# HakimNessah/th_rl

Hardware: AMD Instinct MI355X
Metric: env-steps/sec, 2-agent PD x 1M parallel games (higher is better)
Workload: dtype f32

## Files before the change

th_rl_amd/csrc/thrl_wave_kernel.h:

```cpp
#pragma once
#include <type_traits>
#include "thrl_kernels.h"
#include "thrl_wave_lut.h"

#ifndef THRL_ABLATE
#define THRL_ABLATE 0
#endif

namespace thrl {

constexpr int kAblate = THRL_ABLATE;

typedef unsigned int v2u __attribute__((ext_vector_type(2)));

__device__ __forceinline__ v2u pack_halves(unsigned a, unsigned b) {
    return __builtin_amdgcn_permlane32_swap(a, b, false, false);
}

__device__ __forceinline__ unsigned lds_addr(const void* p) {
    return (unsigned)(uintptr_t)(__attribute__((address_space(3))) const void*)p;
}
template <typename QT>
__device__ __forceinline__ QT lds_load(unsigned addr) {
    typedef __attribute__((address_space(3))) QT lds_t;
    return *(const lds_t*)(uintptr_t)addr;
}
template <typename QT>
__device__ __forceinline__ void lds_store(unsigned addr, QT v) {
    typedef __attribute__((address_space(3))) QT lds_t;
    *(lds_t*)(uintptr_t)addr = v;
}

__device__ __forceinline__ unsigned bperm(unsigned byte_sel, unsigned v) {
    return (unsigned)__builtin_amdgcn_ds_bpermute((int)byte_sel, (int)v);
}

template <int CTRL>
__device__ __forceinline__ double dpp_mov64(double v) {
    const int lo = __double2loint(v), hi = __double2hiint(v);
    return __hiloint2double(__builtin_amdgcn_update_dpp(hi, hi, CTRL, 0xF, 0xF, false),
                            __builtin_amdgcn_update_dpp(lo, lo, CTRL, 0xF, 0xF, false));
}
template <int CTRL>
__device__ __forceinline__ uint32_t dpp_mov32(uint32_t v) {
    return (uint32_t)__builtin_amdgcn_update_dpp((int)v, (int)v, CTRL, 0xF, 0xF, false);
}

__device__ __forceinline__ float group8_allmax(float v) {
    asm("s_nop 1\n\t"
        "v_max_f32_dpp %0, %0, %0 quad_perm:[1,0,3,2] row_mask:0xf bank_mask:0xf\n\t"
        "s_nop 1\n\t"
        "v_max_f32_dpp %0, %0, %0 quad_perm:[2,3,0,1] row_mask:0xf bank_mask:0xf\n\t"
        "s_nop 1\n\t"
        "v_max_f32_dpp %0, %0, %0 row_half_mirror row_mask:0xf bank_mask:0xf"
        : "+v"(v));
    return v;
}
__device__ __forceinline__ double group8_allmax(double v) {
    v = fmax(v, dpp_mov64<0xB1>(v));
    v = fmax(v, dpp_mov64<0x4E>(v));
    v = fmax(v, dpp_mov64<0x141>(v));
    return v;
}
__device__ __forceinline__ void store_where(unsigned long long mask, unsigned addr, float v) {
    unsigned long long save;
    asm volatile("s_mov_b64 %0, exec\n\ts_mov_b64 exec, %1\n\tds_write_b32 %2, %3\n\ts_mov_b64 exec, %0"
                 : "=&s"(save) : "s"(mask), "v"(addr), "v"(v) : "memory");
}
__device__ __forceinline__ void store_where(unsigned long long mask, unsigned addr, double v) {
    unsigned long long save;
    asm volatile("s_mov_b64 %0, exec\n\ts_mov_b64 exec, %1\n\tds_write_b64 %2, %3\n\ts_mov_b64 exec, %0"
                 : "=&s"(save) : "s"(mask), "v"(addr), "v"(v) : "memory");
}
__device__ __forceinline__ float dpp_ror8(float v) { return __builtin_bit_cast(float, dpp_mov32<0x128>(__builtin_bit_cast(uint32_t, v))); }
__device__ __forceinline__ double dpp_ror8(double v) { return dpp_mov64<0x128>(v); }
__device__ __forceinline__ float max_of(float a, float b) { return fmaxf(a, b); }
__device__ __forceinline__ double max_of(double a, double b);
__device__ __forceinline__ float half32_allmax(float v) {
    v = group8_allmax(v);
    v = fmaxf(v, __builtin_bit_cast(float, dpp_mov32<0x140>(__builtin_bit_cast(uint32_t, v))));
    unsigned a = __builtin_bit_cast(unsigned, v), b = a;
    asm("" : "+v"(b));
    const v2u r = __builtin_amdgcn_permlane16_swap(a, b, false, false);
    const unsigned rx = r.x, ry = r.y;
    return fmaxf(__builtin_bit_cast(float, rx), __builtin_bit_cast(float, ry));
}
__device__ __forceinline__ double half32_allmax(double v) {
    v = group8_allmax(v);
    v = fmax(v, dpp_mov64<0x140>(v));
    unsigned lo = (unsigned)__double2loint(v), hi = (unsigned)__double2hiint(v);
    unsigned lo2 = lo, hi2 = hi;
    asm("" : "+v"(lo2), "+v"(hi2));
    const v2u rl = __builtin_amdgcn_permlane16_swap(lo, lo2, false, false);
    const v2u rh = __builtin_amdgcn_permlane16_swap(hi, hi2, false, false);
    const unsigned rlx = rl.x, rly = rl.y, rhx = rh.x, rhy = rh.y;
    return fmax(__hiloint2double((int)rhx, (int)rlx), __hiloint2double((int)rhy, (int)rly));
}
__device__ __forceinline__ double max_of(double a, double b) { return fmax(a, b); }

__device__ __forceinline__ double wave_sum4(double q0, double q1, double q2, double q3, int lane) {
    const bool odd = lane & 1;
    const double k0 = odd ? q1 : q0, k1 = odd ? q3 : q2;
    const double s0 = odd ? q0 : q1, s1 = odd ? q2 : q3;
    const double a0 = k0 + dpp_mov64<0xB1>(s0);
    const double a1 = k1 + dpp_mov64<0xB1>(s1);
    const bool b1 = lane & 2;
    const double kk = b1 ? a1 : a0, ss = b1 ? a0 : a1;
    double v = kk + dpp_mov64<0x4E>(ss);
    v = v + dpp_mov64<0x124>(v);
    v = v + dpp_mov64<0x128>(v);
    {
        unsigned lo = (unsigned)__double2loint(v), hi = (unsigned)__double2hiint(v);
        unsigned lo2 = lo, hi2 = hi;
        asm("" : "+v"(lo2), "+v"(hi2));
        const v2u rl = __builtin_amdgcn_permlane16_swap(lo, lo2, false, false);
        const v2u rh = __builtin_amdgcn_permlane16_swap(hi, hi2, false, false);
        const unsigned rlx = rl.x, rly = rl.y, rhx = rh.x, rhy = rh.y;
        v = __hiloint2double((int)rhx, (int)rlx) + __hiloint2double((int)rhy, (int)rly);
    }
    {
        unsigned lo = (unsigned)__double2loint(v), hi = (unsigned)__double2hiint(v);
        unsigned lo2 = lo, hi2 = hi;
        asm("" : "+v"(lo2), "+v"(hi2));
        const v2u rl = __builtin_amdgcn_permlane32_swap(lo, lo2, false, false);
        const v2u rh = __builtin_amdgcn_permlane32_swap(hi, hi2, false, false);
        const unsigned rlx = rl.x, rly = rl.y, rhx = rh.x, rhy = rh.y;
        v = __hiloint2double((int)rhx, (int)rlx) + __hiloint2double((int)rhy, (int)rly);
    }
    return v;
}

template <int CTRL>
__device__ __forceinline__ uint32_t dpp_src(uint32_t v) {
    return (uint32_t)__builtin_amdgcn_update_dpp(0, (int)v, CTRL, 0xF, 0xF, true);
}

__device__ __forceinline__ float max3_f32(float a, float b, float c) {
    float r;
    asm("v_max3_f32 %0, %1, %2, %3" : "=v"(r) : "v"(a), "v"(b), "v"(c));
    return r;
}
__device__ __forceinline__ uint32_t argmax21_first(unsigned row) {
    float g[7];
#pragma unroll
    for (int k = 0; k < 7; k++)
        g[k] = max3_f32(lds_load<float>(row + 12u * k), lds_load<float>(row + 12u * k + 4u), lds_load<float>(row + 12u * k + 8u));
    const float m = max3_f32(max3_f32(g[0], g[1], g[2]), max3_f32(g[3], g[4], g[5]), g[6]);
    uint32_t c3 = 18u;
#pragma unroll
    for (int k = 5; k >= 0; k--) c3 = (g[k] == m) ? (uint32_t)(3 * k) : c3;
    const unsigned ad = row + 4u * c3;
    const float va = lds_load<float>(ad), vb = lds_load<float>(ad + 4u);
    uint32_t pos = (vb == m) ? 1u : 2u;
    pos = (va == m) ? 0u : pos;
    const float v0 = lds_load<float>(row);
    return (v0 != v0) ? 0u : c3 + pos;
}

__device__ __forceinline__ uint32_t readlane_u(uint32_t v, int lane) {
    return (uint32_t)__builtin_amdgcn_readlane((int)v, lane);
}

__device__ __forceinline__ uint32_t writelane_u(uint32_t old, uint32_t val, int lane) {
    asm("s_mov_b32 m0, %2\n\ts_nop 0\n\tv_writelane_b32 %0, %1, m0" : "+v"(old) : "s"(val), "s"(lane));
    return old;
}

__device__ __forceinline__ uint32_t halves_sum(uint32_t x) {
    uint32_t y;
    asm("v_add_u32_sdwa %0, %1, %1 dst_sel:DWORD dst_unused:UNUSED_PAD src0_sel:WORD_0 src1_sel:WORD_1" : "=v"(y) : "v"(x));
    return y;
}

template <int T0>
__device__ __forceinline__ void chain_group(uint32_t& sq, int& s, uint32_t n0, uint32_t n1, uint32_t n2, uint32_t n3) {
    int s1, s2, s3, s4, pk;
    asm volatile(
        "s_nop 3\n\t"
        "v_readlane_b32 %1, %7, %6\n\t"
        "s_pack_ll_b32_b16 %5, %6, %1\n\t"
        "v_writelane_b32 %0, %5, %11\n\t"
        "s_nop 1\n\t"
        "v_readlane_b32 %2, %8, %1\n\t"
        "s_nop 3\n\t"
        "v_readlane_b32 %3, %9, %2\n\t"
        "s_pack_ll_b32_b16 %5, %2, %3\n\t"
        "v_writelane_b32 %0, %5, %12\n\t"
        "s_nop 1\n\t"
        "v_readlane_b32 %4, %10, %3"
        : "+v"(sq), "=&s"(s1), "=&s"(s2), "=&s"(s3), "=&s"(s4), "=&s"(pk)
        : "s"(s), "v"(n0), "v"(n1), "v"(n2), "v"(n3), "n"(T0), "n"(T0 + 2)
        : "scc");
    s = s4;
}

template <int T0>
__device__ __forceinline__ void chain_group_greedy(uint32_t& sq, int& s, uint32_t g1, uint32_t g2, uint32_t g3, uint32_t g4) {
    int s1, s2, s3, s4, pk;
    asm volatile(
        "s_nop 3\n\t"
        "v_readlane_b32 %1, %7, %6\n\t"
        "v_readlane_b32 %2, %8, %6\n\t"
        "v_readlane_b32 %3, %9, %6\n\t"
        "v_readlane_b32 %4, %10, %6\n\t"
        "s_pack_ll_b32_b16 %5, %6, %1\n\t"
        "v_writelane_b32 %0, %5, %11\n\t"
        "s_pack_ll_b32_b16 %5, %2, %3\n\t"
        "v_writelane_b32 %0, %5, %12"
        : "+v"(sq), "=&s"(s1), "=&s"(s2), "=&s"(s3), "=&s"(s4), "=&s"(pk)
        : "s"(s), "v"(g1), "v"(g2), "v"(g3), "v"(g4), "n"(T0), "n"(T0 + 2)
        : "scc");
    s = s4;
}

template <bool ON> struct GreedyTables {
    __device__ __forceinline__ void build(unsigned) {}
    template <int T0> __device__ __forceinline__ void chain(uint32_t&, int&) const {}
};
template <> struct GreedyTables<true> {
    uint32_t g1, g2, g3, g4;
    __device__ __forceinline__ void build(unsigned lut_addr) {
        g1 = (uint32_t)lds_load<unsigned short>(lut_addr);
        g2 = bperm((g1 & 63u) << 2, g1);
        g3 = bperm((g2 & 63u) << 2, g1);
        g4 = bperm((g2 & 63u) << 2, g2);
    }
    template <int T0> __device__ __forceinline__ void chain(uint32_t& sq, int& s) const { chain_group_greedy<T0>(sq, s, g1, g2, g3, g4); }
};

template <int NRSEG>
__device__ __forceinline__ uint32_t read_row(const uint32_t (&r)[NRSEG], int s) {
    uint32_t v = readlane_u(r[0], s & 63);
    if (NRSEG > 1) {
        const uint32_t h = readlane_u(r[NRSEG - 1], s & 63);
        if (s >= 64) v = h;
    }
    return v;
}
template <int NRSEG>
__device__ __forceinline__ uint32_t gather_row(const uint32_t (&r)[NRSEG], uint32_t row) {
    uint32_t v = bperm((row & 63u) << 2, r[0]);
    if (NRSEG > 1) {
        const uint32_t h = bperm((row & 63u) << 2, r[NRSEG - 1]);
        if (row >= 64u) v = h;
    }
    return v;
}

template <typename QT> struct BlockOps;
template <> struct BlockOps<float> {
    unsigned c1;
    __device__ __forceinline__ void permute(unsigned sel) { c1 = bperm(sel, c1); }
    __device__ __forceinline__ void keep() const { asm volatile("" :: "v"(c1)); }
    __device__ __forceinline__ float value(float nm, float alpha_gamma, float, float) const {
        return __fmaf_rn(alpha_gamma, nm, __builtin_bit_cast(float, c1));
    }
};
template <> struct BlockOps<double> {
    unsigned r_lo, r_hi, t4_lo, t4_hi;
    __device__ __forceinline__ void keep() const { asm volatile("" :: "v"(r_lo), "v"(r_hi), "v"(t4_lo), "v"(t4_hi)); }
    __device__ __forceinline__ void permute(unsigned sel) {
        r_lo = bperm(sel, r_lo); r_hi = bperm(sel, r_hi); t4_lo = bperm(sel, t4_lo); t4_hi = bperm(sel, t4_hi);
    }
    __device__ __forceinline__ double value(double nm, double, double alpha, double gamma) const {
        const double re = __hiloint2double((int)r_hi, (int)r_lo), t4 = __hiloint2double((int)t4_hi, (int)t4_lo);
        const double t2 = __dadd_rn(re, __dmul_rn(gamma, nm));
        return __dadd_rn(t4, __dmul_rn(alpha, t2));
    }
};
template <typename QT> struct Snapshot;
template <> struct Snapshot<float> {
    v2u t4;
    __device__ __forceinline__ void set(float oma0, float ov0, float oma1, float ov1) {
        t4 = pack_halves(__builtin_bit_cast(unsigned, __fmul_rn(oma0, ov0)), __builtin_bit_cast(unsigned, __fmul_rn(oma1, ov1)));
    }
};
template <> struct Snapshot<double> {
    v2u lo, hi;
    __device__ __forceinline__ void set(double oma0, double ov0, double oma1, double ov1) {
        const double x0 = __dmul_rn(oma0, ov0), x1 = __dmul_rn(oma1, ov1);
        lo = pack_halves((unsigned)__double2loint(x0), (unsigned)__double2loint(x1));
        hi = pack_halves((unsigned)__double2hiint(x0), (unsigned)__double2hiint(x1));
    }
};
__device__ __forceinline__ BlockOps<float> make_ops(const Snapshot<float>& s, int k, double r0d, double r1d, float alpha_h) {
    const v2u req = pack_halves(__builtin_bit_cast(unsigned, (float)r0d), __builtin_bit_cast(unsigned, (float)r1d));
    BlockOps<float> o;
    o.c1 = __builtin_bit_cast(unsigned, __fmaf_rn(alpha_h, __builtin_bit_cast(float, k ? req.y : req.x),
                                                  __builtin_bit_cast(float, k ? s.t4.y : s.t4.x)));
    return o;
}
__device__ __forceinline__ BlockOps<double> make_ops(const Snapshot<double>& s, int k, double r0d, double r1d, double) {
    const v2u rl = pack_halves((unsigned)__double2loint(r0d), (unsigned)__double2loint(r1d));
    const v2u rh = pack_halves((unsigned)__double2hiint(r0d), (unsigned)__double2hiint(r1d));
    BlockOps<double> o;
    o.r_lo = k ? rl.y : rl.x; o.r_hi = k ? rh.y : rh.x;
    o.t4_lo = k ? s.lo.y : s.lo.x; o.t4_hi = k ? s.hi.y : s.hi.x;
    return o;
}
template <typename QT> struct HP;
template <> struct HP<float> {
    static __device__ __forceinline__ float gamma(const AgentParams& p) { return p.gamma_f; }
    static __device__ __forceinline__ float alpha(const AgentParams& p) { return p.alpha_f; }
    static __device__ __forceinline__ float one_minus_alpha(const AgentParams& p) { return p.one_minus_alpha_f; }
    static __device__ __forceinline__ float from_double(double x) { return (float)x; }
    static __device__ __forceinline__ float product(float a, float g) { return __fmul_rn(a, g); }
};
template <> struct HP<double> {
    static __device__ __forceinline__ double gamma(const AgentParams& p) { return p.gamma; }
    static __device__ __forceinline__ double alpha(const AgentParams& p) { return p.alpha; }
    static __device__ __forceinline__ double one_minus_alpha(const AgentParams& p) { return p.one_minus_alpha; }
    static __device__ __forceinline__ double from_double(double x) { return x; }
    static __device__ __forceinline__ double product(double, double) { return 0.0; }
};

template <typename QT, int RDN, bool FIXED_POINTS, bool PER2>
__device__ __forceinline__ void replay_group(int gi, uint32_t P, int lane_base, int nsub, const BlockOps<QT>& ops, unsigned wo,
                                             unsigned rd_base, unsigned row_shift, unsigned my_step,
                                             unsigned row_bytes, QT alpha_gamma, QT alpha, QT gamma, bool upper_half,
                                             int block_step0, int replay_from) {
    const int first = replay_from - (block_step0 + gi * 4);
    if (first >= 4) return;
    const uint32_t sP = readlane_u(P, lane_base + gi * 4);
    const int nv = min(4, nsub - gi * 4);
    unsigned ad0;
    asm("v_mad_u32_u24 %0, %1, %2, %3" : "=v"(ad0) : "v"((sP >> row_shift) & 0x7Fu), "s"(row_bytes), "v"(rd_base));
    unsigned ad[RDN];
#pragma unroll
    for (int i = 0; i < RDN; i++) ad[i] = ad0 + (unsigned)(i * sizeof(QT));
    if (FIXED_POINTS && PER2 && (sP >> 31) && nv == 4 && first <= 0 && !(kAblate & 256) && (sP & 0x7Fu) != ((sP >> 7) & 0x7Fu)) {
        const unsigned ca0 = readlane_u(wo, gi), ca1 = readlane_u(wo, 32 + gi);
        const unsigned cb0 = readlane_u(wo, 8 + gi), cb1 = readlane_u(wo, 40 + gi);
        const bool odd = (my_step & 1u) != 0u;
// ... 261 lines not shown
        if (SWEEP && a.sw_gamma) gamma_h = HP<QT>::from_double(a.sw_gamma[(size_t)half * a.G + g]);
        if (SWEEP && a.sw_alpha) {
            alpha_h = HP<QT>::from_double(a.sw_alpha[(size_t)half * a.G + g]);
            oma0 = HP<QT>::from_double(__dsub_rn(1.0, a.sw_alpha[g]));
            oma1 = HP<QT>::from_double(__dsub_rn(1.0, a.sw_alpha[(size_t)a.G + g]));
        }
        double epsg0 = 0.0, epsg1 = 0.0;
        const bool sw_eps_on = SWEEP && a.sw_eps != nullptr;
        if (sw_eps_on) { epsg0 = a.sw_eps[g]; epsg1 = a.sw_eps[(size_t)a.G + g]; }
        const QT ag_h = HP<QT>::product(alpha_h, gamma_h);
        const double eend0 = (SWEEP && a.sw_eps_end) ? a.sw_eps_end[g] : p0.eps_end;
        const double eend1 = (SWEEP && a.sw_eps_end) ? a.sw_eps_end[(size_t)a.G + g] : p1.eps_end;
        const double estep0 = (SWEEP && a.sw_eps_step) ? a.sw_eps_step[g] : p0.eps_step;
        const double estep1 = (SWEEP && a.sw_eps_step) ? a.sw_eps_step[(size_t)a.G + g] : p1.eps_step;
        const double noise_prob_g = (SWEEP && a.sw_noise_prob) ? a.sw_noise_prob[g] : a.env.noise_prob;

        {
            const QT* s0 = q0 + lo * A;
            const QT* s1 = q1 + lo * A;
            const int n = W * A;
            for (int k0 = 0; k0 < n; k0 += 512) {
                QT v0[8], v1[8];
#pragma unroll
                for (int j = 0; j < 8; j++) {
                    const int k = min(k0 + j * 64 + lane, n - 1);
                    v0[j] = s0[k]; v1[j] = s1[k];
                }
#pragma unroll
                for (int j = 0; j < 8; j++) {
                    const int k = k0 + j * 64 + lane;
                    if (k < n) { tab0[k] = v0[j]; tab1[k] = v1[j]; }
                }
            }
        }
        int sp = __builtin_amdgcn_readfirstlane(encode32(price0, p0));
        int st = __builtin_amdgcn_readfirstlane(encode64(price0, p0));
        sp = min(max(sp, 0), a.rows - 1);
        st = min(max(st, 0), a.rows - 1);
        int spill0 = -1, spill1 = -1, sp_l, st_l;
        if (sp >= lo && sp < lo + W) sp_l = sp - lo; else { spill0 = sp; sp_l = W; }
        if (st == sp) st_l = sp_l;
        else if (st >= lo && st < lo + W) st_l = st - lo;
        else { spill1 = st; st_l = W + 1; }

        {
            if (spill0 >= 0 && lane < A) {
                tab0[W * A + lane] = q0[spill0 * A + lane];
                tab1[W * A + lane] = q1[spill0 * A + lane];
            }
            if (spill1 >= 0 && lane < A) {
                tab0[(W + 1) * A + lane] = q0[spill1 * A + lane];
                tab1[(W + 1) * A + lane] = q1[spill1 * A + lane];
            }
        }
        __builtin_amdgcn_wave_barrier();

        int s = sp_l | (st_l << 8);
        double last_price = price0;
        for (int e = 0; e < a.n_episodes; e += epk) {
            const uint32_t eg = (uint32_t)(a.first_episode + (uint64_t)e);

            uint32_t AM[NRSEG], R[NRSEG];
            uint32_t G0q = 0u, G1q = 0u;
#pragma unroll
            for (int k = 0; k < NRSEG; k++) {
                const int row = min(lane + 64 * k, W + 1);
                const QT* r0 = tab0 + row * A;
                const QT* r1 = tab1 + row * A;
                QT b0 = r0[0], b1 = r1[0];
                uint32_t i0 = 0, i1 = 0;
                if (kAblate & 16) {
                } else if (kArgmax21 && A == 21) {
                    i0 = argmax21_first(tab0_off + (unsigned)row * 84u);
                    i1 = argmax21_first(tab1_off + (unsigned)row * 84u);
                } else if (A == 21) {
#pragma unroll
                    for (int j = 1; j < 21; j++) {
                        const QT v0 = r0[j], v1 = r1[j];
                        if (v0 > b0) { b0 = v0; i0 = j; }
                        if (v1 > b1) { b1 = v1; i1 = j; }
                    }
                } else {
#pragma unroll 4
                    for (int j = 1; j < A; j++) {
                        const QT v0 = r0[j], v1 = r1[j];
                        if (v0 > b0) { b0 = v0; i0 = j; }
                        if (v1 > b1) { b1 = v1; i1 = j; }
                    }
                }
                if (kAblate & 16) { i0 = (uint32_t)(lane * 5) % (uint32_t)A; i1 = (uint32_t)(lane * 3) % (uint32_t)A; }
                AM[k] = i0 | (i1 << 8);
                R[k] = (i0 * (uint32_t)A * 2u) | (i1 << 17);
                if constexpr (AFFINE) {
                    G0q = i0 * ((uint32_t)a.aff_m0 * 0x01010101u);
                    G1q = i1 * ((uint32_t)a.aff_m1 * 0x01010101u);
                }
            }
            GreedyTables<GREEDY && NRSEG == 1> gt;
            gt.build(halves_sum(R[0]) + lut_ns_lds);

            uint32_t seq[NSEG], rwv[NSEG];
            unsigned explored_segs = 0u;
            double nav[NSEG];
#pragma unroll
            for (int seg = 0; seg < NSEG; seg++) {
                int n = min(64, T - seg * 64);
                asm volatile("" : "+s"(n));
                uint32_t rw;
                nav[seg] = 0.0;
                const int tcl = min(seg * 64 + lane, T - 1);
                const int ep = epk == 1 ? 0 : tcl / Tenv;
                const uint32_t st_in_ep = (uint32_t)(tcl - ep * Tenv);
                double eps0, eps1;
                if (sw_eps_on) { eps0 = epsg0; eps1 = epsg1; }
                else if (epk == 1) { eps0 = a.eps[e][0]; eps1 = a.eps[e][1]; }
                else { eps0 = a.eps[e + ep][0]; eps1 = a.eps[e + ep][1]; }
                if (a.inj_u) {
                    const int tt = tcl;
                    const size_t k = (((size_t)e * Tenv + tt) * 2) * (size_t)a.G + (size_t)g;
                    const uint32_t ex0 = a.inj_u[k] < eps0 ? 1u : 0u;
                    const uint32_t ex1 = a.inj_u[k + a.G] < eps1 ? 2u : 0u;
                    const uint32_t c0 = min((uint32_t)(uint8_t)a.inj_choice[k], (uint32_t)(A - 1));
                    const uint32_t c1 = min((uint32_t)(uint8_t)a.inj_choice[k + a.G], (uint32_t)(A - 1));
                    rw = ex0 | ex1 | (c0 << 8) | (c1 << 16);
                } else if (kAblate & 8) {
                    const uint32_t h = (uint32_t)(lane * 2654435761u) ^ eg;
                    rw = (h & 3u) | (((h >> 4) % (uint32_t)A) << 8) | (((h >> 12) % (uint32_t)A) << 16);
                } else {
                    uint32_t seed_lo = (uint32_t)a.seed, seed_hi = (uint32_t)(a.seed >> 32);
                    asm volatile("" : "+s"(seed_lo), "+s"(seed_hi));
                    const uint64_t seed_here = ((uint64_t)seed_hi << 32) | seed_lo;
                    const u32x4 x = draw(seed_here, gid, eg + (uint32_t)ep, st_in_ep, 0u);
                    const uint32_t ex0 = u01_32(x.x) < eps0 ? 1u : 0u;
                    const uint32_t ex1 = u01_32(x.z) < eps1 ? 2u : 0u;
                    rw = ex0 | ex1 | (__umulhi(x.y, (uint32_t)A) << 8) | (__umulhi(x.w, (uint32_t)A) << 16);
                }
                if (NOISE) {
                    double nu, na;
                    if (a.inj_u) {
                        const size_t k = ((size_t)e * Tenv + tcl) * (size_t)a.G + (size_t)g;
                        nu = a.inj_noise_u[k]; na = a.inj_noise_a[k];
                    } else {
                        const u32x4 xn = draw(a.seed, gid, eg + (uint32_t)ep, st_in_ep, kStreamNoise);
                        nu = u01_32(xn.x);
                        na = __dadd_rn(a.env.noise_lo, __dmul_rn(__dsub_rn(a.env.a, a.env.noise_lo), u01_32(xn.y)));
                    }
                    if (nu < noise_prob_g) rw |= 4u;
                    nav[seg] = na;
                }
                rwv[seg] = rw;
                if constexpr (AFFINE) {
                    seq[seg] = play_affine(seg, n, lane, rw, G0q, G1q, mk_addr, a.aff_c, a.aff_m0, a.aff_m1, s);
                } else {
                const uint32_t Mv = ((rw & 1u) ? 0u : 0xFFFFu) | ((rw & 2u) ? 0u : 0xFFFF0000u);
                const uint32_t Kv = lut_ns_lds + 2u * (((rw & 1u) ? ((rw >> 8) & 0xFFu) * (uint32_t)A : 0u) +
                                                      ((rw & 2u) ? ((rw >> 16) & 0xFFu) : 0u));
                const unsigned long long noisy_steps = NOISE ? __ballot((rw & 4u) != 0u) : 0ull;
                unsigned long long busy_groups = 0ull;
                if (GREEDY && __ballot((rw & 3u) != 0u && seg * 64 + lane < T) != 0ull) explored_segs |= 1u << seg;
                if (GREEDY && NRSEG == 1) {
                    busy_groups = __ballot((rw & (NOISE ? 7u : 3u)) != 0u || seg * 64 + lane >= T);
                    busy_groups |= busy_groups >> 1;
                    busy_groups |= busy_groups >> 2;
                }
                constexpr bool greedy_copy = GREEDY && NRSEG == 1 && !(kAblate & 6);
                auto build = [&](int t, uint32_t (&out)[NRSEG], bool may_be_noisy) {
                    const int tl = t;
                    if (NOISE && may_be_noisy) {
                        if ((noisy_steps >> tl) & 1ull) {
                            const uint32_t w = readlane_u(rw, tl);
                            const double na = __hiloint2double(__builtin_amdgcn_readlane(__double2hiint(nav[seg]), tl),
                                                               __builtin_amdgcn_readlane(__double2loint(nav[seg]), tl));
                            const uint32_t c0 = (w >> 8) & 0xFFu, c1 = (w >> 16) & 0xFFu;
#pragma unroll
                            for (int k = 0; k < NRSEG; k++) {
                                const uint32_t a0r = (w & 1u) ? c0 : (AM[k] & 0xFFu), a1r = (w & 2u) ? c1 : (AM[k] >> 8);
                                const double Q = __dadd_rn(lut_aq[a0r], lut_aq[A + a1r]);
                                double pr = __dsub_rn(na, __dmul_rn(a.env.b, Q));
                                if (!(pr > 0.0)) pr = 0.0;
                                const int r32 = min(max(encode32_fast(pr, p0) - lo, 0), W - 1);
                                const int r64 = min(max(encode64_fast(pr, p0) - lo, 0), W - 1);
                                out[k] = (uint32_t)(r32 | (r64 << 8));
                            }
                            return;
                        }
                    }
                    if (kAblate & 4) {
#pragma unroll
                        for (int k = 0; k < NRSEG; k++) out[k] = (R[k] >> 17) + (uint32_t)(t & 3);
                        return;
                    }
                    const uint32_t sM = readlane_u(Mv, tl), sK = readlane_u(Kv, tl);
#pragma unroll
                    for (int k = 0; k < NRSEG; k++) out[k] = lds_load<unsigned short>(halves_sum(R[k] & sM) + sK);
                };
                uint32_t sq = 0, sq_tail = 0;
                auto chain4 = [&](auto t0c, const int n, const uint32_t (&tab)[4][NRSEG], const bool all_greedy = false) {
                    constexpr int t0 = decltype(t0c)::value;
                    if (kAblate & 2) {
                        asm volatile("" :: "v"(tab[0][0]), "v"(tab[1][0]), "v"(tab[2][0]), "v"(tab[3][0]));
                        sq_tail = (uint32_t)min(lane, W - 1) * 0x101u;
                        return;
                    }
                    if (NRSEG == 1 && t0 + 4 <= n) {
                        s = __builtin_amdgcn_readfirstlane(s);
                        if (GREEDY && all_greedy) gt.template chain<t0>(sq, s);
                        else chain_group<t0>(sq, s, tab[0][0], tab[1][0], tab[2][0], tab[3][0]);
                        return;
                    }
                    s = __builtin_amdgcn_readfirstlane(s);
#pragma unroll
                    for (int j = 0; j < 4; j++) {
                        if (t0 + j < n) {
                            sq_tail = writelane_u(sq_tail, (uint32_t)s, t0 + j);
                            s = (int)read_row<NRSEG>(tab[j], s & 0xFF);
                        }
                    }
                };
                uint32_t ta[4][NRSEG], tb[4][NRSEG];
                v2u mkr[4] = {v2u{0u, 0u}, v2u{0u, 0u}, v2u{0u, 0u}, v2u{0u, 0u}};
                if (kLdsMK) {
                    if (lane < 32) lds_store<v2u>(mk_addr + 8u * (unsigned)lane, v2u{Mv, Kv});
                    __builtin_amdgcn_wave_barrier();
#pragma unroll
                    for (int j = 0; j < 4; j++) mkr[j] = lds_load<v2u>(mk_addr + 8u * (unsigned)j);
                }
                auto build4 = [&](int t0, uint32_t (&tab)[4][NRSEG]) {
                    if (kLdsMK) {
                        unsigned ad[4];
#pragma unroll
                        for (int j = 0; j < 4; j++) ad[j] = halves_sum(R[0] & mkr[j].x) + mkr[j].y;
#pragma unroll
                        for (int j = 0; j < 4; j++) tab[j][0] = lds_load<unsigned short>(ad[j]);
                        if (t0 == 28) {
                            if (lane >= 32) lds_store<v2u>(mk_addr + 8u * (unsigned)(lane - 32), v2u{Mv, Kv});
                            __builtin_amdgcn_wave_barrier();
                        }
#pragma unroll
                        for (int j = 0; j < 4; j++) mkr[j] = lds_load<v2u>(mk_addr + 8u * (unsigned)(min(t0 + 4 + j, 63) & 31));
                        return;
                    }
                    if (NOISE && ((noisy_steps >> t0) & 0xFull)) {
#pragma unroll
                        for (int j = 0; j < 4; j++) build(t0 + j, tab[j], true);
                    } else {
#pragma unroll
                        for (int j = 0; j < 4; j++) build(t0 + j, tab[j], false);
                    }
                };
#define THRL_PLAY2(G, N_)                                                                    \
                if ((G) * 4 < (N_)) {                                                        \
                    if ((G) * 4 + 4 < (N_)) build4((G) * 4 + 4, tb);                         \
                    chain4(std::integral_constant<int, (G) * 4>(), (N_), ta);                \
                    if ((G) * 4 + 4 < (N_)) {                                                \
                        if ((G) * 4 + 8 < (N_)) build4((G) * 4 + 8, ta);                     \
                        chain4(std::integral_constant<int, (G) * 4 + 4>(), (N_), tb);        \
                    }                                                                        \
                }
#define THRL_PLAY16(N_)                                                                      \
                THRL_PLAY2(0, N_) THRL_PLAY2(2, N_) THRL_PLAY2(4, N_) THRL_PLAY2(6, N_)      \
                THRL_PLAY2(8, N_) THRL_PLAY2(10, N_) THRL_PLAY2(12, N_) THRL_PLAY2(14, N_)
#define THRL_PLAY2G(G, N_)                                                                   \
                if ((G) * 4 + 8 <= (N_) && g0 &&                                             \
                    !(busy_groups & (((G) * 4 + 8 < 64 ? 0x110ull : 0x10ull) << ((G) * 4)))) {   \
                     \
                    chain4(std::integral_constant<int, (G) * 4>(), (N_), ta, true);          \
                    chain4(std::integral_constant<int, (G) * 4 + 4>(), (N_), tb, true);      \
                } else if ((G) * 4 < (N_)) {                                                 \
                    const bool g1 = !((busy_groups >> ((G) * 4 + 4)) & 1ull);                \
                    if ((G) * 4 + 4 < (N_) && !g1) build4((G) * 4 + 4, tb);                  \
                    chain4(std::integral_constant<int, (G) * 4>(), (N_), ta, g0);            \
                    if ((G) * 4 + 4 < (N_)) {                                                \
                        g0 = (G) * 4 + 8 < 64 && !((busy_groups >> (((G) * 4 + 8) & 63)) & 1ull);   \
                        if ((G) * 4 + 8 < (N_) && !g0) build4((G) * 4 + 8, ta);              \
                        chain4(std::integral_constant<int, (G) * 4 + 4>(), (N_), tb, g1);    \
                    }                                                                        \
                }
#define THRL_PLAY16G(N_)                                                                         \
                THRL_PLAY2G(0, N_) THRL_PLAY2G(2, N_) THRL_PLAY2G(4, N_) THRL_PLAY2G(6, N_)      \
                THRL_PLAY2G(8, N_) THRL_PLAY2G(10, N_) THRL_PLAY2G(12, N_) THRL_PLAY2G(14, N_)
                if (greedy_copy) {
                    bool g0 = !(busy_groups & 1ull);
                    if (!g0) build4(0, ta);
                    if (n == 64) { THRL_PLAY16G(64) } else if (n == 36) { THRL_PLAY16G(36) } else { THRL_PLAY16G(n) }
                } else {
                    build4(0, ta);
                    if (n == 64) { THRL_PLAY16(64) } else if (n == 36) { THRL_PLAY16(36) } else { THRL_PLAY16(n) }
                }
#undef THRL_PLAY16G
#undef THRL_PLAY2G
#undef THRL_PLAY16
#undef THRL_PLAY2
                {
                    const int packed_end = (NRSEG == 1 && !(kAblate & 2)) ? (n & ~3) : 0;
                    const uint32_t prev = dpp_mov32<0x111>(sq);
                    const uint32_t un = (lane & 1) ? (prev >> 16) : (sq & 0xFFFFu);
                    seq[seg] = lane < packed_end ? un : sq_tail;
                }
                }
            }
            const int s_end = s;

            uint32_t act[NSEG];
            Snapshot<QT> snap[NSEG];
#pragma unroll
            for (int seg = 0; seg < NSEG; seg++) {
                const int tt = seg * 64 + lane;
                const bool valid = tt < T;
                const uint32_t my_s = seq[seg] & 0xFFu;
                const uint32_t my_train = (seq[seg] >> 8) & 0xFFu;
                const uint32_t rw = rwv[seg];
                const uint32_t gam = gather_row<NRSEG>(AM, my_s);
                uint32_t a0 = (rw & 1u) ? ((rw >> 8) & 0xFFu) : (gam & 0xFFu);
                uint32_t a1 = (rw & 2u) ? ((rw >> 16) & 0xFFu) : (gam >> 8);
                uint32_t nxt = (uint32_t)__shfl_down((int)seq[seg], 1, 64);
                if (seg + 1 < NSEG) { if (lane == 63) nxt = readlane_u(seq[seg + 1 < NSEG ? seg + 1 : seg], 0); }
                const uint32_t ns = (tt + 1 < T) ? ((nxt >> 8) & 0xFFu) : ((uint32_t)s_end >> 8);
                uint32_t srow = my_train;
                if (!valid) { a0 = 0; a1 = 0; srow = 0; }
                snap[seg].set(oma0, tab0[srow * A + a0], oma1, tab1[srow * A + a1]);
                act[seg] = a0 | (a1 << 8) | (srow << 16) | (ns << 24);
            }
            __builtin_amdgcn_wave_barrier();

            double lr0 = 0.0, lr1 = 0.0, la0 = 0.0, la1 = 0.0;
            auto log_into = [&](int epi, double q0, double q1, double q2, double q3, bool first) {
                double v = (kAblate & 64) ? q0 + q1 + q2 + q3 : wave_sum4(q0, q1, q2, q3, lane);
                if ((lane & 3) < 2) v = __ddiv_rn(v, inv_T_den);
                if constexpr (LOG) {
                    double *grl, *gal;
                    game_log_ptrs<WaveArgs>(grl, gal);
                    if (grl && lane < 2) {
                        double* p = grl + ((size_t)epi * 2 + lane) * a.G + g;
                        *p = first ? v : *p + v;
                    }
                    if (gal && (lane >> 1) == 1) {
                        double* p = gal + ((size_t)epi * 2 + (lane & 1)) * a.G + g;
                        *p = first ? v : *p + v;
                    }
                }
                const long long vq = __double2ll_rn(__dmul_rn(v, log_scale));
                if ((lane >> 2) == (epi & 15)) { if (epi < 16) acc += vq; else acc_hi += vq; }
            };
#pragma unroll
            for (int seg = 0; seg < NSEG; seg++) {
                const int tt = seg * 64 + lane;
                const bool valid = tt < T;
                const uint32_t a0 = act[seg] & 0xFFu, a1 = (act[seg] >> 8) & 0xFFu;
                const uint32_t srow = (act[seg] >> 16) & 0xFFu;
                const double aq0 = lut_aq[a0], aq1 = lut_aq[A + a1];
                const double a_eff = (NOISE && (rwv[seg] & 4u)) ? nav[seg] : a.env.a;
                double price = __dsub_rn(a_eff, __dmul_rn(a.env.b, __dadd_rn(aq0, aq1)));
                if (!(price > 0.0)) price = 0.0;
                const double r0d = __dmul_rn(price, aq0);
                const double r1d = __dmul_rn(price, aq1);
                if (seg == NSEG - 1) {
                    const int ll = T - 1 - seg * 64;
                    last_price = __hiloint2double(__builtin_amdgcn_readlane(__double2hiint(price), ll),
                                                  __builtin_amdgcn_readlane(__double2loint(price), ll));
                }
                const v2u woq = pack_halves(tab0_off + (srow * A + a0) * (unsigned)sizeof(QT),
                                            tab1_off + (srow * A + a1) * (unsigned)sizeof(QT));
                if (epk == 1) {
                    if (valid) {
                        lr0 += r0d; lr1 += r1d;
                        la0 += lut_sct[a0]; la1 += lut_sct[A + a1];
                    }
                } else {
                    const int ep_l = min(tt, T - 1) / Tenv;
                    const int j0 = (seg * 64) / Tenv, j1 = (min(T, seg * 64 + 64) - 1) / Tenv;
                    const double s0 = lut_sct[a0], s1 = lut_sct[A + a1];
                    for (int j = j0; j <= j1; j++) {
                        const bool m = valid && ep_l == j;
                        log_into(e + j, m ? r0d : 0.0, m ? r1d : 0.0, m ? s0 : 0.0, m ? s1 : 0.0, j * Tenv >= seg * 64);
                    }
                }
                if (a.counter && !(kAblate & 32))
                    a.tlog[(((size_t)wave_gid * kWaveMaxEpisodes + e) * NSEG + seg) * 64 + lane] =
                        valid ? act[seg] : 0xFFFFFFFFu;

                uint32_t P;
                bool any_fixed;
                if (kAblate & 128) { P = (act[seg] >> 24) * 0x204081u; any_fixed = false; }
                else if constexpr (kMaskSched) {
                    const uint32_t w = act[seg];
                    const uint32_t d = (w >> 24) ^ ((w >> 16) & 0xFFu);
                    uint32_t x0 = w ^ dpp_src<0x00>(w), x1 = w ^ dpp_src<0x55>(w), x2 = w ^ dpp_src<0xAA>(w);
                    asm("" : "+v"(x0), "+v"(x1), "+v"(x2));
                    auto hz = [&](uint32_t x) -> unsigned long long {
                        const uint32_t xr = (x >> 16) & 0xFFu;
                        return __ballot((((x & 0xFFu) * ((x >> 8) & 0xFFu)) | xr) == 0u) | __ballot(xr == d);
                    };
                    const unsigned long long H0 = hz(x0), H1 = hz(x1), H2 = hz(x2);
                    const unsigned long long M = 0x1111111111111111ull;
                    const unsigned long long C1 = (H0 >> 1) & M;
                    const unsigned long long C2 = ((H1 >> 2) | ((H0 >> 2) & ~C1)) & M;
                    const unsigned long long C3 = ((H2 >> 3) | (((H1 >> 3) | ((H0 >> 3) & ~C1)) & ~C2)) & M;
                    const unsigned long long F = (__ballot((x0 | x1 | x2) == 0u) >> 3) & __ballot(d == 0u) & M;
                    const unsigned long long sched = C1 | (C2 << 1) | (C3 << 2) | (F << 3);
                    any_fixed = F != 0ull;
                    uint32_t rows = (w >> 24) << (7u * ((uint32_t)lane & 3u));
                    rows |= dpp_src<0xB1>(rows);
                    rows |= dpp_src<0x4E>(rows);
                    P = ((uint32_t)(sched >> lane) << 28) | rows;
                } else {
                    const uint32_t w = act[seg];
                    const uint32_t b0 = dpp_mov32<0x00>(w), b1 = dpp_mov32<0x55>(w), b2 = dpp_mov32<0xAA>(w),
                                   b3 = dpp_mov32<0xFF>(w);
                    const uint32_t qp = (uint32_t)lane & 3u;
                    auto hz = [&](uint32_t bi, uint32_t i) -> uint32_t {
                        const bool raw = (w >> 24) == ((bi >> 16) & 0xFFu);
                        const bool waw = ((w >> 16) & 0xFFu) == ((bi >> 16) & 0xFFu) &&
                                         ((w & 0xFFu) == (bi & 0xFFu) || ((w >> 8) & 0xFFu) == ((bi >> 8) & 0xFFu));
                        return (qp > i && (raw || waw)) ? 1u : 0u;
                    };
                    const uint32_t hzw = hz(b0, 0u) | (hz(b1, 1u) << 1) | (hz(b2, 2u) << 2);
                    const uint32_t h1 = dpp_mov32<0x55>(hzw), h2 = dpp_mov32<0xAA>(hzw), h3 = dpp_mov32<0xFF>(hzw);
                    const uint32_t c1 = h1 & 1u;
                    const uint32_t c2 = ((h2 >> 1) & 1u) | ((c1 ^ 1u) & h2 & 1u);
                    const uint32_t c3 = ((h3 >> 2) & 1u) | ((c2 ^ 1u) & (((h3 >> 1) & 1u) | ((c1 ^ 1u) & h3 & 1u)));
                    bool quad_quiet = true;
                    if (NOISE) quad_quiet = ((__ballot((rwv[seg] & 4u) != 0u) >> (lane & 60)) & 0xFull) == 0ull;
                    const uint32_t same4 = ((quad_quiet && b0 == b1 && b1 == b2 && b2 == b3 && (b0 >> 24) == ((b0 >> 16) & 0xFFu)) ||
                                            (GREEDY && b0 == b2 && b1 == b3 && (b0 >> 24) == ((b1 >> 16) & 0xFFu) &&
                                             (b1 >> 24) == ((b0 >> 16) & 0xFFu) && (b0 >> 24) != (b1 >> 24))) ? 1u : 0u;
                    P = (b0 >> 24) | ((b1 >> 24) << 7) | ((b2 >> 24) << 14) | ((b3 >> 24) << 21) |
                        ((c1 | (c2 << 1) | (c3 << 2)) << 28) | (same4 << 31);
                    any_fixed = __ballot((P >> 31) != 0u) != 0ull;
                }

                bool seg_done = false;
                if (GREEDY && !(kAblate & 257) && !((explored_segs >> seg) & 1u)) {
                    const int nseg = min(64, T - seg * 64);
                    const uint32_t w = act[seg];
                    const uint32_t w1 = dpp_mov32<0x138>(w), w2 = dpp_mov32<0x138>(w1);
                    const uint32_t w3 = dpp_mov32<0x138>(w2), w4 = dpp_mov32<0x138>(w3);
                    const bool in_seg = lane < nseg;
                    const int period = __ballot(in_seg && lane >= 1 && w != w1) == 0ull ? 1
                                     : __ballot(in_seg && lane >= 2 && w != w2) == 0ull ? 2
                                     : __ballot(in_seg && lane >= 3 && w != w3) == 0ull ? 3
                                     : __ballot(in_seg && lane >= 4 && w != w4) == 0ull ? 4 : 0;
                    if (period > 0 && nseg >= period) {
                        uint32_t W[4];
#pragma unroll
                        for (int j = 0; j < 4; j++) W[j] = readlane_u(w, j);
                        bool ok = true;
#pragma unroll
                        for (int j = 0; j < 4; j++)
                            if (j < period) {
                                const uint32_t nxt_row = (W[(j + 1 < period) ? j + 1 : 0] >> 16) & 0xFFu;
                                ok = ok && (W[j] >> 24) == nxt_row;
#pragma unroll
                                for (int i = 0; i < j; i++) ok = ok && ((W[i] >> 16) & 0xFFu) != ((W[j] >> 16) & 0xFFu);
                            }
                        if (ok) {
                            seg_done = true;
                            const BlockOps<QT> ops0 = make_ops(snap[seg], 0, r0d, r1d, alpha_h);
                            const unsigned tabh = half ? tab1_off : tab0_off;
                            if (period == 1) cyclic_segment<QT, 1>(ops0, woq.x, W, nseg, lane, tabh, A, row_bytes, ag_h, alpha_h, gamma_h);
                            else if (period == 2) cyclic_segment<QT, 2>(ops0, woq.x, W, nseg, lane, tabh, A, row_bytes, ag_h, alpha_h, gamma_h);
                            else if (period == 3) cyclic_segment<QT, 3>(ops0, woq.x, W, nseg, lane, tabh, A, row_bytes, ag_h, alpha_h, gamma_h);
                            else cyclic_segment<QT, 4>(ops0, woq.x, W, nseg, lane, tabh, A, row_bytes, ag_h, alpha_h, gamma_h);
                            __builtin_amdgcn_wave_barrier();
                        }
                    }
                }
#pragma unroll
                for (int k = 0; k < 2; k++) {
                    if (GREEDY && seg_done) break;
                    int nsub = __builtin_amdgcn_readfirstlane(min(32, T - seg * 64 - k * 32));
                    asm volatile("" : "+s"(nsub));
                    if (nsub <= 0) break;
                    BlockOps<QT> ops = make_ops(snap[seg], k, r0d, r1d, alpha_h);
                    ops.permute(perm_sel);
                    const unsigned wo = bperm(perm_sel, k ? woq.y : woq.x);
#define THRL_REPLAY(RDN_, FP_) replay_block<QT, RDN_, FP_, kUnrollReplay && RDN_ == 3, GREEDY>(P, k * 32, nsub, ops, wo, rd_base, row_shift, my_step, row_bytes, \
                                                          ag_h, alpha_h, gamma_h, half != 0, seg * 64 + k * 32, replay_from)
                    if (A > 24)      { if (any_fixed) THRL_REPLAY(4, true); else THRL_REPLAY(4, false); }
                    else if (A >= 3) { if (any_fixed) THRL_REPLAY(3, true); else THRL_REPLAY(3, false); }
                    else             { if (any_fixed) THRL_REPLAY(2, true); else THRL_REPLAY(2, false); }
#undef THRL_REPLAY
                }
            }

            if (epk == 1) log_into(e, lr0, lr1, la0, la1, true);
            if (SWEEP) {
                epsg0 = __dadd_rn(eend0, __dmul_rn(__dsub_rn(epsg0, eend0), estep0));
                epsg1 = __dadd_rn(eend1, __dmul_rn(__dsub_rn(epsg1, eend1), estep1));
            }
        }

        {
            QT* d0 = q0 + lo * A;
            QT* d1 = q1 + lo * A;
            const int n = W * A;
            for (int k = lane; k < n; k += 64) { d0[k] = tab0[k]; d1[k] = tab1[k]; }
            if (spill0 >= 0 && lane < A) {
                q0[spill0 * A + lane] = tab0[W * A + lane];
                q1[spill0 * A + lane] = tab1[W * A + lane];
            }
            if (spill1 >= 0 && lane < A) {
                q0[spill1 * A + lane] = tab0[(W + 1) * A + lane];
                q1[spill1 * A + lane] = tab1[(W + 1) * A + lane];
            }
            if (lane == 0 && a.n_episodes > 0) a.state[g] = last_price;
            if (lane == 0 && sw_eps_on) { a.sw_eps[g] = epsg0; a.sw_eps[(size_t)a.G + g] = epsg1; }
        }
        __builtin_amdgcn_wave_barrier();

        if (a.counter && !(kAblate & 32)) {
            const int cells = (W + 2) * A;
            const int hw = (cells + 1) >> 1;
            typedef unsigned __attribute__((may_alias)) hist_u32;
            hist_u32* hist = reinterpret_cast<hist_u32*>(tab0);
            __builtin_amdgcn_fence(__ATOMIC_SEQ_CST, "wavefront");
            for (int k = lane; k < 2 * hw; k += 64) hist[k] = 0u;
            __builtin_amdgcn_wave_barrier();
            const int n_cycles = a.n_episodes / epk;
            for (int c0 = 0; c0 < n_cycles; c0 += 4) {
                unsigned w[4][NSEG];
#pragma unroll
                for (int j = 0; j < 4; j++)
#pragma unroll
                    for (int seg = 0; seg < NSEG; seg++)
                        w[j][seg] = __hip_atomic_load(
                            &a.tlog[(((size_t)wave_gid * kWaveMaxEpisodes + min(c0 + j, n_cycles - 1) * epk) * NSEG + seg) * 64 + lane],
                            __ATOMIC_RELAXED, __HIP_MEMORY_SCOPE_AGENT);
#pragma unroll
                for (int j = 0; j < 4; j++)
#pragma unroll
                    for (int seg = 0; seg < NSEG; seg++) {
                        const unsigned ww = w[j][seg];
                        if (c0 + j < n_cycles && ww != 0xFFFFFFFFu && seg * 64 + lane >= replay_from) {
                            const unsigned srow = (ww >> 16) & 0xFFu;
                            const unsigned c0_ = srow * (unsigned)A + (ww & 0xFFu);
                            const unsigned c1_ = srow * (unsigned)A + ((ww >> 8) & 0xFFu);
                            __hip_atomic_fetch_add(&hist[c0_ >> 1], 1u << ((c0_ & 1u) << 4), __ATOMIC_RELAXED, __HIP_MEMORY_SCOPE_WAVEFRONT);
                            __hip_atomic_fetch_add(&hist[hw + (c1_ >> 1)], 1u << ((c1_ & 1u) << 4), __ATOMIC_RELAXED, __HIP_MEMORY_SCOPE_WAVEFRONT);
                        }
                    }
            }
            __builtin_amdgcn_wave_barrier();
            int32_t* cw0 = a.counter + (int64_t)g * a.stride + p0.table_off;
            int32_t* cw1 = a.counter + (int64_t)g * a.stride + p1.table_off;
            const int nwin = W * A;
            for (int k0 = 0; k0 < nwin; k0 += 512) {
                int32_t c0v[8], c1v[8];
#pragma unroll
                for (int j = 0; j < 8; j++) {
                    const int k = min(k0 + j * 64 + lane, nwin - 1);
                    c0v[j] = cw0[lo * A + k]; c1v[j] = cw1[lo * A + k];
                }
#pragma unroll
                for (int j = 0; j < 8; j++) {
                    const int k = k0 + j * 64 + lane;
                    if (k < nwin) {
                        const unsigned n0 = (hist[k >> 1] >> ((k & 1) << 4)) & 0xFFFFu;
                        const unsigned n1 = (hist[hw + (k >> 1)] >> ((k & 1) << 4)) & 0xFFFFu;
                        if (n0) cw0[lo * A + k] = c0v[j] + (int32_t)n0;
                        if (n1) cw1[lo * A + k] = c1v[j] + (int32_t)n1;
                    }
                }
            }
            if (lane < 2 * A) {
                const int which = lane >= A, col = lane - which * A;
                const int grow_ = which ? spill1 : spill0;
                const int k = nwin + lane;
                if (grow_ >= 0) {
                    const unsigned n0 = (hist[k >> 1] >> ((k & 1) << 4)) & 0xFFFFu;
                    const unsigned n1 = (hist[hw + (k >> 1)] >> ((k & 1) << 4)) & 0xFFFFu;
                    if (n0) cw0[grow_ * A + col] += (int32_t)n0;
                    if (n1) cw1[grow_ * A + col] += (int32_t)n1;
                }
            }
            __builtin_amdgcn_fence(__ATOMIC_SEQ_CST, "wavefront");
            __builtin_amdgcn_wave_barrier();
        }
    }
    a.partial[(size_t)wave_gid * 128 + lane] = acc;
    a.partial[(size_t)wave_gid * 128 + 64 + lane] = acc_hi;
}

template <typename QT, int NSEG, int NRSEG, bool NOISE, bool SWEEP, bool CYCLE, bool GREEDY, bool LOG, bool AFFINE = false>
static int launch_wave_t(const WaveArgs& a, int grid, int block, size_t lds, hipStream_t s) {
    auto kern = k_wave_episodes<QT, NSEG, NRSEG, NOISE, SWEEP, CYCLE, GREEDY, LOG, AFFINE>;
    if (lds > 64 * 1024) {
        const hipError_t e = hipFuncSetAttribute(reinterpret_cast<const void*>(kern),
                                                 hipFuncAttributeMaxDynamicSharedMemorySize, (int)lds);
        if (e != hipSuccess) return (int)e;
    }
    hipLaunchKernelGGL(kern, dim3(grid), dim3(block), lds, s, a);
    return (int)hipGetLastError();
}

template <typename QT, bool NOISE, bool SWEEP, bool CYCLE, bool GREEDY, bool LOG>
static int launch_wave_nl(const WaveArgs& a, int grid, int block, size_t lds, hipStream_t s) {
    const int nseg = (a.T * a.epk + 63) / 64;
    const int nrseg = (a.win_rows + 2 + 63) / 64;
    if (nrseg == 1) {
        switch (nseg) {
            case 1: return launch_wave_t<QT, 1, 1, NOISE, SWEEP, CYCLE, GREEDY, LOG>(a, grid, block, lds, s);
            case 2: return launch_wave_t<QT, 2, 1, NOISE, SWEEP, CYCLE, GREEDY, LOG>(a, grid, block, lds, s);
            case 3: return launch_wave_t<QT, 3, 1, NOISE, SWEEP, CYCLE, GREEDY, LOG>(a, grid, block, lds, s);
            case 4: return launch_wave_t<QT, 4, 1, NOISE, SWEEP, CYCLE, GREEDY, LOG>(a, grid, block, lds, s);
        }
    } else if (nrseg == 2) {
        switch (nseg) {
            case 1: return launch_wave_t<QT, 1, 2, NOISE, SWEEP, CYCLE, GREEDY, LOG>(a, grid, block, lds, s);
            case 2: return launch_wave_t<QT, 2, 2, NOISE, SWEEP, CYCLE, GREEDY, LOG>(a, grid, block, lds, s);
            case 3: return launch_wave_t<QT, 3, 2, NOISE, SWEEP, CYCLE, GREEDY, LOG>(a, grid, block, lds, s);
            case 4: return launch_wave_t<QT, 4, 2, NOISE, SWEEP, CYCLE, GREEDY, LOG>(a, grid, block, lds, s);
        }
    }
    return -1;
}

template <typename QT, bool NOISE, bool SWEEP, bool CYCLE, bool GREEDY = false>
static int launch_wave_n(const WaveArgs& a, int grid, int block, size_t lds, hipStream_t s) {
    if (a.game_reward_log || a.game_action_log) return launch_wave_nl<QT, NOISE, SWEEP, CYCLE, GREEDY, true>(a, grid, block, lds, s);
    return launch_wave_nl<QT, NOISE, SWEEP, CYCLE, GREEDY, false>(a, grid, block, lds, s);
}

}
```

Baseline: 43.70 billion.

## Precompute LDS cell offsets in trace log and use 32-bit histogram counters

Each step now computes a packed pair of LDS word offsets for both agents' table cells once. That pair is reused for the snapshot loads, the pack_halves addresses and the trace log, and steps before replay_from are masked when logged rather than at replay time. The replay histogram switches from packed 16-bit halves to one 32-bit counter per cell, incremented with a simple LDS atomic at the logged offset, which removes per-entry decode arithmetic. A DPP row shift replaces a shfl_down. The new scheme assumes tab1 sits at a fixed offset of (W+2)*A cells after tab0 and that offsets fit in 16 bits, so it breaks silently if either assumption does not hold.

Result: faster. 44.50 billion (median of 6 runs) (+1.8%).

```diff
diff --git a/th_rl_amd/csrc/thrl_wave_kernel.h b/th_rl_amd/csrc/thrl_wave_kernel.h
--- a/th_rl_amd/csrc/thrl_wave_kernel.h
+++ b/th_rl_amd/csrc/thrl_wave_kernel.h
@@ -29,6 +29,17 @@
 __device__ __forceinline__ void lds_store(unsigned addr, QT v) {
     typedef __attribute__((address_space(3))) QT lds_t;
     *(lds_t*)(uintptr_t)addr = v;
+}
+
+__device__ __forceinline__ void lds_inc(unsigned addr) {
+    typedef unsigned __attribute__((may_alias)) u32_alias;
+    typedef __attribute__((address_space(3))) u32_alias lds_u32;
+    __hip_atomic_fetch_add((lds_u32*)(uintptr_t)addr, 1u, __ATOMIC_RELAXED, __HIP_MEMORY_SCOPE_WAVEFRONT);
+}
+__device__ __forceinline__ void lds_zero8(unsigned addr) {
+    typedef unsigned long long __attribute__((may_alias)) u64_alias;
+    typedef __attribute__((address_space(3))) u64_alias lds_u64;
+    *(lds_u64*)(uintptr_t)addr = 0ull;
 }
 
 __device__ __forceinline__ unsigned bperm(unsigned byte_sel, unsigned v) {
@@ -896,6 +907,8 @@
             const int s_end = s;
 
             uint32_t act[NSEG];
+            uint32_t cwv[NSEG];
+            constexpr unsigned kCellScale = (unsigned)sizeof(QT) / 4u;
             Snapshot<QT> snap[NSEG];
 #pragma unroll
             for (int seg = 0; seg < NSEG; seg++) {
@@ -907,12 +920,16 @@
                 const uint32_t gam = gather_row<NRSEG>(AM, my_s);
                 uint32_t a0 = (rw & 1u) ? ((rw >> 8) & 0xFFu) : (gam & 0xFFu);
                 uint32_t a1 = (rw & 2u) ? ((rw >> 16) & 0xFFu) : (gam >> 8);
-                uint32_t nxt = (uint32_t)__shfl_down((int)seq[seg], 1, 64);
+                uint32_t nxt = dpp_mov32<0x130>(seq[seg]);
                 if (seg + 1 < NSEG) { if (lane == 63) nxt = readlane_u(seq[seg + 1 < NSEG ? seg + 1 : seg], 0); }
                 const uint32_t ns = (tt + 1 < T) ? ((nxt >> 8) & 0xFFu) : ((uint32_t)s_end >> 8);
                 uint32_t srow = my_train;
                 if (!valid) { a0 = 0; a1 = 0; srow = 0; }
-                snap[seg].set(oma0, tab0[srow * A + a0], oma1, tab1[srow * A + a1]);
+                const uint32_t rowc = __umul24(srow, (uint32_t)A);
+                const uint32_t cw = ((rowc + a0) | ((rowc + a1 + (uint32_t)((W + 2) * A)) << 16)) << 2;
+                cwv[seg] = cw;
+                snap[seg].set(oma0, lds_load<QT>(tab0_off + (cw & 0xFFFFu) * kCellScale),
+                              oma1, lds_load<QT>(tab0_off + (cw >> 16) * kCellScale));
                 act[seg] = a0 | (a1 << 8) | (srow << 16) | (ns << 24);
             }
             __builtin_amdgcn_wave_barrier();
@@ -941,7 +958,6 @@
                 const int tt = seg * 64 + lane;
                 const bool valid = tt < T;
                 const uint32_t a0 = act[seg] & 0xFFu, a1 = (act[seg] >> 8) & 0xFFu;
-                const uint32_t srow = (act[seg] >> 16) & 0xFFu;
                 const double aq0 = lut_aq[a0], aq1 = lut_aq[A + a1];
                 const double a_eff = (NOISE && (rwv[seg] & 4u)) ? nav[seg] : a.env.a;
                 double price = __dsub_rn(a_eff, __dmul_rn(a.env.b, __dadd_rn(aq0, aq1)));
@@ -953,8 +969,7 @@
                     last_price = __hiloint2double(__builtin_amdgcn_readlane(__double2hiint(price), ll),
                                                   __builtin_amdgcn_readlane(__double2loint(price), ll));
                 }
-                const v2u woq = pack_halves(tab0_off + (srow * A + a0) * (unsigned)sizeof(QT),
-                                            tab1_off + (srow * A + a1) * (unsigned)sizeof(QT));
+                const v2u woq = pack_halves(tab0_off + (cwv[seg] & 0xFFFFu) * kCellScale, tab0_off + (cwv[seg] >> 16) * kCellScale);
                 if (epk == 1) {
                     if (valid) {
                         lr0 += r0d; lr1 += r1d;
@@ -971,7 +986,7 @@
                 }
                 if (a.counter && !(kAblate & 32))
                     a.tlog[(((size_t)wave_gid * kWaveMaxEpisodes + e) * NSEG + seg) * 64 + lane] =
-                        valid ? act[seg] : 0xFFFFFFFFu;
+                        (valid && tt >= replay_from) ? cwv[seg] : 0xFFFFFFFFu;
 
                 uint32_t P;
                 bool any_fixed;
@@ -1104,11 +1119,10 @@
 
         if (a.counter && !(kAblate & 32)) {
             const int cells = (W + 2) * A;
-            const int hw = (cells + 1) >> 1;
             typedef unsigned __attribute__((may_alias)) hist_u32;
             hist_u32* hist = reinterpret_cast<hist_u32*>(tab0);
             __builtin_amdgcn_fence(__ATOMIC_SEQ_CST, "wavefront");
-            for (int k = lane; k < 2 * hw; k += 64) hist[k] = 0u;
+            for (int k = lane; k < cells; k += 64) lds_zero8(tab0_off + 8u * (unsigned)k);
             __builtin_amdgcn_wave_barrier();
             const int n_cycles = a.n_episodes / epk;
             for (int c0 = 0; c0 < n_cycles; c0 += 4) {
@@ -1125,12 +1139,9 @@
 #pragma unroll
                     for (int seg = 0; seg < NSEG; seg++) {
                         const unsigned ww = w[j][seg];
-                        if (c0 + j < n_cycles && ww != 0xFFFFFFFFu && seg * 64 + lane >= replay_from) {
-                            const unsigned srow = (ww >> 16) & 0xFFu;
-                            const unsigned c0_ = srow * (unsigned)A + (ww & 0xFFu);
-                            const unsigned c1_ = srow * (unsigned)A + ((ww >> 8) & 0xFFu);
-                            __hip_atomic_fetch_add(&hist[c0_ >> 1], 1u << ((c0_ & 1u) << 4), __ATOMIC_RELAXED, __HIP_MEMORY_SCOPE_WAVEFRONT);
-                            __hip_atomic_fetch_add(&hist[hw + (c1_ >> 1)], 1u << ((c1_ & 1u) << 4), __ATOMIC_RELAXED, __HIP_MEMORY_SCOPE_WAVEFRONT);
+                        if (c0 + j < n_cycles && ww != 0xFFFFFFFFu) {
+                            lds_inc(tab0_off + (ww & 0xFFFFu));
+                            lds_inc(tab0_off + (ww >> 16));
                         }
                     }
             }
@@ -1149,8 +1160,7 @@
                 for (int j = 0; j < 8; j++) {
                     const int k = k0 + j * 64 + lane;
                     if (k < nwin) {
-                        const unsigned n0 = (hist[k >> 1] >> ((k & 1) << 4)) & 0xFFFFu;
-                        const unsigned n1 = (hist[hw + (k >> 1)] >> ((k & 1) << 4)) & 0xFFFFu;
+                        const unsigned n0 = hist[k], n1 = hist[cells + k];
                         if (n0) cw0[lo * A + k] = c0v[j] + (int32_t)n0;
                         if (n1) cw1[lo * A + k] = c1v[j] + (int32_t)n1;
                     }
@@ -1161,8 +1171,7 @@
                 const int grow_ = which ? spill1 : spill0;
                 const int k = nwin + lane;
                 if (grow_ >= 0) {
-                    const unsigned n0 = (hist[k >> 1] >> ((k & 1) << 4)) & 0xFFFFu;
-                    const unsigned n1 = (hist[hw + (k >> 1)] >> ((k & 1) << 4)) & 0xFFFFu;
+                    const unsigned n0 = hist[k], n1 = hist[cells + k];
                     if (n0) cw0[grow_ * A + col] += (int32_t)n0;
                     if (n1) cw1[grow_ * A + col] += (int32_t)n1;
                 }
```
